# microsoft/timewarp

Measured on AMD Instinct MI355X. Metric: MH-accepted samples/sec (whole node), alanine-dipeptide kernel_transformer_nvp, higher is better.
Workload: dtype f16x3 (split-fp16 operands, 3 MFMAs per fp32 product, fp32 accumulate)

## Files before the change

### include/timewarp_hip.h

```cpp
#ifndef TIMEWARP_HIP_H
#define TIMEWARP_HIP_H

#include <stddef.h>
#include <stdint.h>

#ifdef __cplusplus
extern "C" {
#endif

#define TW_ABI_VERSION 8

typedef enum {
  TW_OK = 0,
  TW_ERR_INVALID = -1,
  TW_ERR_HIP = -2,
  TW_ERR_WORKSPACE = -3,
  TW_ERR_NO_DEVICE = -4
} tw_status;

typedef struct {
  int32_t variant;
  int32_t n_coupling;
  int32_t n_layers;
  int32_t d_model;
// ... 180 lines not shown
                           const tw_forcefield* ff, const tw_mh_options* opt, const tw_mh_draws* draws,
                           const int32_t* atom_types, const uint8_t* masked, int32_t n_atoms, const float* x_coords,
                           const float* x_velocs, float* cur_velocs, float* zy_coords, float* zy_velocs, float* u,
                           float* new_coords, float* new_velocs, float* out_stats, uint8_t* out_accepted, int32_t* result,
                           int64_t n_proposals, int64_t n_chains, void* workspace, int64_t workspace_bytes, void* stream);
int tw_mh_draw_chains(const tw_flow_desc* desc, const float* raw, const tw_mh_draws* draws, float* z_coords, float* z_velocs,
                      float* u, float* velocs, int64_t n_proposals, int64_t n_chains, int32_t n_atoms, void* stream);

int tw_chirality_changed(const float* coords, const int32_t* centres, const float* reference_signs,
                         int32_t n_centres, uint8_t* out_changed, int64_t n_rows, int32_t n_atoms,
                         void* stream);

int tw_profile_begin(void);
int tw_profile_end(double* total_ms, int64_t* launches);

int tw_probe_mfma_clock(int32_t workgroups, int32_t iters, int64_t* cycles, double* ms, void* stream);

const char* tw_last_netblock_kernel(void);

const char* tw_last_attention_kernel(void);

const char* tw_flow_selected_kernel(const tw_flow_desc* desc, int32_t n_atoms, int64_t n_rows, int32_t path);

int tw_flow_nonfinite(int32_t reset, int32_t* out_flag);

#define TW_DEBUG_EXP_NO_WEIGHT_DMA (1 << 0)
#define TW_DEBUG_EXP_NO_BARRIERS (1 << 1)
#define TW_DEBUG_DUMP_ATTENTION (1 << 2)
#define TW_DEBUG_COMPILED_CPP (1 << 3)
#define TW_DEBUG_SECTION_STAMPS (1 << 4)
#define TW_DEBUG_SEPARATE_COUPLING (1 << 5)
#define TW_DEBUG_EXP_DENSE_NO_SOFTMAX (1 << 6)
#define TW_DEBUG_EXP_DENSE_NO_QKV_LDS (1 << 7)
#define TW_DEBUG_KEEP_PADDING (1 << 10)
#define TW_DEBUG_EXP_DENSE_NO_ATTENTION (1 << 11)
#define TW_DEBUG_PER_SECTION (1 << 12)
#define TW_DEBUG_ENC_WITH_DUMPS (1 << 13)
#define TW_DEBUG_NEVER_WIDE (1 << 14)
#define TW_DEBUG_ALWAYS_WIDE (1 << 15)
#define TW_DEBUG_ALWAYS_NT4 (1 << 16)
#define TW_DEBUG_NEVER_NT4 (1 << 17)
#define TW_DEBUG_WIDE_FIVE_GROUP_WINDOWS (1 << 18)
#define TW_DEBUG_WIDE_XT_BYTE_STORES (1 << 19)
#define TW_DEBUG_NEVER_PAIRED (1 << 20)
#define TW_DEBUG_PER_OP_ROWWISE (1 << 21)
#define TW_DEBUG_ENERGY_MAIN_STREAM (1 << 22)
#define TW_DEBUG_ENERGY_SIDE_STREAM (1 << 23)
#define TW_DEBUG_PER_OP_UNFUSED (1 << 24)
#define TW_DEBUG_FOLD_GEMM_SEPARATE (1 << 25)
#define TW_DEBUG_FOLD_ONE_WG_PER_TILE (1 << 26)
#define TW_DEBUG_FOLD_LN_SEPARATE (1 << 27)
#define TW_DEBUG_IO_GEMM_PAIRS (1 << 28)
#define TW_DEBUG_TOKENS_NT3 (1 << 29)
#define TW_DEBUG_TOKENS_NT4 (1 << 30)
#define TW_DEBUG_SDPA_SCALAR (-0x7fffffff - 1)
int tw_debug_set_flags(int flags);

int tw_debug_netblock(const tw_flow_desc* desc, const float* raw, const float* packed,
                      int32_t coupling, int32_t net, const int32_t* atom_types,
                      const float* x_coords, const float* x_velocs, const uint8_t* masked,
                      int64_t n_cond, const float* z_other, int64_t n_rows, int32_t n_atoms,
                      int32_t path, float* dump, void* workspace, int64_t workspace_bytes,
                      void* stream);

#ifdef __cplusplus
}
// ... 3 lines not shown
```

### timewarp_amd/_lib.py

```python
from __future__ import annotations

import ctypes as C
import enum
import os
from typing import Optional

import torch

from . import build as _build

_LIB: Optional[C.CDLL] = None

TW_PATH_AUTO, TW_PATH_FUSED, TW_PATH_SIMPLE, TW_PATH_FUSED_H3, TW_PATH_FUSED_H1, TW_PATH_SIMPLE_H3 = 0, 1, 2, 3, 4, 5


class DebugFlag(enum.IntFlag):

    EXP_NO_WEIGHT_DMA = 1 << 0
    EXP_NO_BARRIERS = 1 << 1
    DUMP_ATTENTION = 1 << 2
    COMPILED_CPP = 1 << 3
    SECTION_STAMPS = 1 << 4
    SEPARATE_COUPLING = 1 << 5
    EXP_DENSE_NO_SOFTMAX = 1 << 6
    EXP_DENSE_NO_QKV_LDS = 1 << 7
    KEEP_PADDING = 1 << 10
    EXP_DENSE_NO_ATTENTION = 1 << 11
    PER_SECTION = 1 << 12
    ENC_WITH_DUMPS = 1 << 13
    NEVER_WIDE = 1 << 14
    ALWAYS_WIDE = 1 << 15
    ALWAYS_NT4 = 1 << 16
    NEVER_NT4 = 1 << 17
    WIDE_FIVE_GROUP_WINDOWS = 1 << 18
    WIDE_XT_BYTE_STORES = 1 << 19
    NEVER_PAIRED = 1 << 20
    PER_OP_ROWWISE = 1 << 21
    ENERGY_MAIN_STREAM = 1 << 22
    ENERGY_SIDE_STREAM = 1 << 23
    PER_OP_UNFUSED = 1 << 24
    FOLD_GEMM_SEPARATE = 1 << 25
    FOLD_ONE_WG_PER_TILE = 1 << 26
    FOLD_LN_SEPARATE = 1 << 27
    IO_GEMM_PAIRS = 1 << 28
    TOKENS_NT3 = 1 << 29
    TOKENS_NT4 = 1 << 30
    SDPA_SCALAR = 1 << 31


def debug_word(flags) -> int:
    word = int(flags) & 0xFFFFFFFF
    return word - (1 << 32) if word & (1 << 31) else word


class FlowDesc(C.Structure):

    _fields_ = [
        ("variant", C.c_int32),
        ("n_coupling", C.c_int32),
        ("n_layers", C.c_int32),
        ("d_model", C.c_int32),
        ("d_ff", C.c_int32),
        ("d_hidden", C.c_int32),
        ("d_emb", C.c_int32),
        ("n_heads", C.c_int32),
        ("d_rff", C.c_int32),
        ("n_elements", C.c_int32),
        ("pos_mod2", C.c_int32),
        ("displacement", C.c_int32),
        ("ignore_cond_velocity", C.c_int32),
        ("normalise", C.c_int32),
        ("ln_eps", C.c_float),
        ("cheb_order", C.c_int32),
        ("cheb_force_zero", C.c_int32),
        ("range_flag", C.c_void_p),
        ("max_radius", C.c_float),
        ("n_hidden", C.c_int32),
    ]


# ... 177 lines not shown
```

### timewarp_amd/csrc/tw_netblock_h3.hip

```cpp
#include <utility>
#include <vector>

#include "tw_common.h"

namespace tw {

typedef float f4 __attribute__((ext_vector_type(4)));
typedef _Float16 h8 __attribute__((ext_vector_type(8)));
typedef _Float16 h4 __attribute__((ext_vector_type(4)));
typedef unsigned u4 __attribute__((ext_vector_type(4)));
typedef unsigned u2 __attribute__((ext_vector_type(2)));

#define H3_NT 3
#define H3_FFN_SPLIT 4
#define H3_TOK (16 * H3_NT)
#define H3_XT 48
#define H3_XT_IMG 1536
#define H3_PAIR_BYTES 2048
#define H3_STAGE_PAIRS 4
#define H3_STAGE_TILE_BYTES 8192
#define H3_STAGE_BYTES 9216
#define H3_RING 5
#define H3_XT_BYTES (128 * H3_XT * 2)
#define H3_WAVE_LDS (2 * H3_XT_BYTES)
// ... 512 lines not shown
    *(h8*)(base + lane * 16) = hi;
    *(h8*)(base + 1024 + lane * 16) = lo;
  }
}

struct H3Params {
  const char* packed;
  int64_t net_stride_bytes;
  int64_t stages;
  int64_t side_in2b, side_layers, side_layer_size, side_out2b, side_scales;
  const float* emb;
  const int32_t* types;
  const float* xc;
  const float* xv;
  const float* z_other;
  const char* sfrag;
  int sfrag_shared;
  int64_t sf_variant_bytes;
  int windowed;
  const float* rff;
  int d_rff;
  int win[4];
  float* out[2];
  float* dump;
  int64_t n_rows, n_cond;
  int V, mpw, nblocks;
  int ng;
  int P;
  int H, n_layers, ff_chunks, hid_chunks, d_emb;
  float eps;
  int net_sel;
  int debug;
  const uint8_t* masked;
  PrevCoupling prev;
};
#define H3_OPS(...)                                                                                                    \
  : [cur] "+&s"(cur), [gn] "+&v"(gn) : [ring] "s"(ring), [wave] "s"(wave), [priv] "s"(priv_lds), __VA_ARGS__ :
#define H3_IN_WIDE [xt] "s"(xt_lds), [win] "s"(win)
#define H3_IN_MASK0 [m0l] "v"(m0l), [m0h] "v"(m0h)
#define H3_IN_MASK12 [m1l] "v"(m1l), [m1h] "v"(m1h), [m2l] "v"(m2l), [m2h] "v"(m2h)
#define H3_OPS_IO H3_OPS([chunks] "s"(chunks))
#define H3_IN_ATTN [heads] "s"(heads), [sf] "v"(sfp)
#define H3_OPS_ATTN H3_OPS(H3_IN_ATTN)
#define H3_OPS_ATTN_WIDE H3_OPS(H3_IN_ATTN, H3_IN_WIDE)
#define H3_OPS_ATTN_DENSE H3_OPS([sl] "s"(sl_lds), H3_IN_MASK0, H3_IN_MASK12)
#define H3_OPS_ENC_V                                                                                                   \
  H3_OPS([heads] "s"(heads), [chunks] "s"(chunks), [layers] "s"(layers), [sf] "v"(sfp), [sfstride] "s"(sfstride),      \
         [side] "v"(sidep), [sidestride] "s"(sidestride), [sl] "s"(sl_lds), [scales] "s"(scp), [eps] "s"(eps),        \
         [padm] "v"(padmask), [padt] "s"(pad_tiles), [dump] "v"(stamp_base), [stampen] "s"(stampen))
#define H3_IN_ENC_S_SF                                                                                                 \
  [heads] "s"(heads), [chunks] "s"(chunks), [layers] "s"(layers), [sf] "s"(sf_u), [sfstride] "s"(sfstride_lo),         \
      [sfstridehi] "s"(sfstride_hi)
#define H3_IN_ENC_S_SIDE                                                                                               \
  [side] "s"(side_u), [sidestride] "s"(sidestride32), [sl] "s"(sl_lds), [scales] "s"(scales_u), [eps] "s"(eps),        \
      [padm] "v"(padmask), [padt] "s"(pad_tiles), [dump] "s"(dump_u), [stampen] "s"(stampen)
#define H3_OPS_ENC_S H3_OPS(H3_IN_ENC_S_SF, H3_IN_ENC_S_SIDE)
#define H3_OPS_ENC_S_WIDE H3_OPS(H3_IN_ENC_S_SF, H3_IN_ENC_S_SIDE, H3_IN_WIDE)
#define H3_OPS_ENC_DENSE4 H3_OPS([chunks] "s"(chunks), [layers] "s"(layers), H3_IN_ENC_S_SIDE, H3_IN_MASK0)
#define H3_OPS_ENC_DENSE3 H3_OPS([chunks] "s"(chunks), [layers] "s"(layers), H3_IN_ENC_S_SIDE, H3_IN_MASK0, H3_IN_MASK12)
__device__ __forceinline__ void h3_load_sf4(const char* p, u4 (&r)[16]) {
  asm volatile(
      "global_load_dwordx4 %0, %16, off\n\t"
      "global_load_dwordx4 %1, %16, off offset:1024\n\t"
      "global_load_dwordx4 %2, %16, off offset:2048\n\t"
      "global_load_dwordx4 %3, %16, off offset:3072\n\t"
      "global_load_dwordx4 %4, %17, off\n\t"
// ... 31 lines not shown
  for (int jt = 0; jt < NT; ++jt) acc[jt] = mfma32(ah, b.l[jt], acc[jt]);
#pragma unroll
  for (int jt = 0; jt < NT; ++jt) acc[jt] = mfma32(al, b.h[jt], acc[jt]);
}

__device__ __forceinline__ void split_pair(float a, float b, unsigned& hi, unsigned& lo) {
  float ta, tb;
  asm("v_cvt_pk_f16_f32 %0, %4, %5\n\t"
      "v_fma_mix_f32 %2, %0, -1.0, %4 op_sel_hi:[1,0,0]\n\t"
      "v_fma_mix_f32 %3, %0, -1.0, %5 op_sel:[1,0,0] op_sel_hi:[1,0,0]\n\t"
      "v_cvt_pk_f16_f32 %1, %2, %3"
      : "=&v"(hi), "=&v"(lo), "=&v"(ta), "=&v"(tb)
      : "v"(a), "v"(b));
}

__device__ __forceinline__ void split8(const f4 a, const f4 b, h8& hi, h8& lo) {
  unsigned h0, h1, h2, h3, l0, l1, l2, l3;
  split_pair(a[0], a[1], h0, l0);
  split_pair(a[2], a[3], h1, l1);
  split_pair(b[0], b[1], h2, l2);
  split_pair(b[2], b[3], h3, l3);
  hi = __builtin_bit_cast(h8, (u4){h0, h1, h2, h3});
  lo = __builtin_bit_cast(h8, (u4){l0, l1, l2, l3});
}

__device__ __forceinline__ void split4(const f4 a, h4& hi, h4& lo) {
  unsigned h0, h1, l0, l1;
  split_pair(a[0], a[1], h0, l0);
  split_pair(a[2], a[3], h1, l1);
  hi = __builtin_bit_cast(h4, (u2){h0, h1});
  lo = __builtin_bit_cast(h4, (u2){l0, l1});
}

__device__ __forceinline__ void h3_swap16(float& a, float& b) {
  asm("s_nop 1\n\tv_permlane16_swap_b32 %0, %1" : "+v"(a), "+v"(b));
}
__device__ __forceinline__ void h3_swap32(float& a, float& b) {
  asm("s_nop 1\n\tv_permlane32_swap_b32 %0, %1" : "+v"(a), "+v"(b));
}
__device__ __forceinline__ float h3_quad_max(float v) {
  float a = v, b = v;
  h3_swap16(a, b);
  a = b = fmaxf(a, b);
  h3_swap32(a, b);
  return fmaxf(a, b);
}
__device__ __forceinline__ float h3_quad_sum(float v) {
  float a = v, b = v;
  h3_swap16(a, b);
  a = b = a + b;
  h3_swap32(a, b);
  return a + b;
}

__device__ __forceinline__ float h3_xor_sum(float v) { return h3_quad_sum(v); }

template <int NT, int KS>
__device__ __forceinline__ void to_bop(const f4 (&x)[2 * KS][NT], BOp<NT> (&b)[KS]) {
#pragma unroll
  for (int ks = 0; ks < KS; ++ks)
#pragma unroll
    for (int jt = 0; jt < NT; ++jt) split8(x[2 * ks][jt], x[2 * ks + 1][jt], b[ks].h[jt], b[ks].l[jt]);
}

__device__ __forceinline__ void h3_load_sf3(const char* p16, const char* p8, u4 (&a)[3], u4 (&b)[3], u2 (&c)[3], u2 (&d)[3]) {
  asm volatile(
// ... 283 lines not shown
      const char* src = (const char*)(side + p.side_layers) + lane * 16;
      char* dst = lds + SIDE_LDS_OFFSET;
#pragma unroll
      for (int i = 0; i < SIDE_CHUNKS; ++i)
        __builtin_amdgcn_global_load_lds((const __attribute__((address_space(1))) void*)(src + i * 1024),
                                         (__attribute__((address_space(3))) void*)(dst + i * 1024), 16, 0, 0);
    }
  }
  pipe.start_issue();

  const float sc_in2 = scales[1], sc_out2 = scales[2 + 3 * p.n_layers + 1];
  f4 bb_in2[8];
#pragma unroll
  for (int ot = 0; ot < 8; ++ot) bb_in2[ot] = *(const f4*)(side + p.side_in2b + 4 * g + 16 * ot);
  const f4 bb_out2 = *(const f4*)(side + p.side_out2b + 4 * g);

  int64_t tok_row[NT];
  int64_t tok_cond[NT];
  int tok_atom[NT];
  const unsigned inv_v = (65536u + (unsigned)p.P - 1u) / (unsigned)p.P;
  const bool cond_shared = p.n_cond == 1, cond_per_row = p.n_cond >= p.n_rows;
#pragma unroll
  for (int jt = 0; jt < NT; ++jt) {
    const int t = slot0 + 16 * jt + i16;
    const int q = (int)(((unsigned)t * inv_v) >> 16);
    const int64_t n = row0 + q;
    const int atom = t - q * p.P;
    const bool ok = active && q < p.mpw && n < p.n_rows && atom < p.V;
    tok_row[jt] = ok ? n : -1;
    tok_cond[jt] = !ok || cond_shared ? 0 : (cond_per_row ? n : n % p.n_cond);
    tok_atom[jt] = ok ? atom : 0;
  }
  float zo[NT][3];
  {
    float part[NT];
    bool bad = false;
#pragma unroll
    for (int jt = 0; jt < NT; ++jt) {
      const int64_t n = tok_row[jt];
      part[jt] = 0.f;
#pragma unroll
      for (int k = 0; k < 3; ++k) zo[jt][k] = 0.f;
      if (n < 0) continue;
      const int64_t idx = (n * p.V + tok_atom[jt]) * 3;
      if (p.prev.s_raw) {
        float ld = 0.f;
#pragma unroll
        for (int k = 0; k < 3; ++k) {
          const float sr = p.prev.s_raw[idx + k], shift = p.prev.t[idx + k];
          const float scale = expf(sr);
          bad |= !(isfinite(sr) && isfinite(shift));
          const float z = p.prev.z_in[idx + k];
          zo[jt][k] = p.prev.reverse ? (z - shift) / scale : z * scale + shift;
          ld += logf(scale);
        }
        part[jt] = p.masked[tok_cond[jt] * p.V + tok_atom[jt]] ? 0.f : ld;
        if (net == 0 && g == 0) {
#pragma unroll
          for (int k = 0; k < 3; ++k) p.prev.z_out[idx + k] = zo[jt][k];
        }
      } else {
#pragma unroll
        for (int k = 0; k < 3; ++k) zo[jt][k] = p.z_other[idx + k];
      }
    }
    if constexpr (WIDE) {
      if (p.prev.s_raw) {
// ... 9 lines not shown
        __builtin_amdgcn_s_barrier();
        if (net == 0 && wave == 0 && lane < p.mpw) {
          const int64_t n = row0 + lane;
          if (n < p.n_rows) {
            float acc = 0.f;
            for (int a = 0; a < p.V; ++a) acc += scr[lane * p.P + a];
            p.prev.delta_logp[n] -= p.prev.reverse ? -acc : acc;
          }
        }
        asm volatile("s_waitcnt lgkmcnt(0)" ::: "memory");
        __builtin_amdgcn_s_barrier();
      }
    } else
    if (p.prev.s_raw && net == 0) {
      if (bad) atomicOr(p.prev.nonfinite, 1);
      float* scr = (float*)xt_hi;
      if (g == 0) {
#pragma unroll
        for (int jt = 0; jt < NT; ++jt) scr[16 * jt + i16] = part[jt];
      }
      if (lane < p.mpw) {
        const int64_t n = (int64_t)blk * p.mpw + lane;
        if (active && n < p.n_rows) {
          float acc = 0.f;
          for (int a = 0; a < p.V; ++a) acc += scr[lane * p.V + a];
          p.prev.delta_logp[n] -= p.prev.reverse ? -acc : acc;
        }
      }
    }
  }
  const unsigned long long t_pro1 = (p.debug & TW_DEBUG_SECTION_STAMPS) ? __builtin_readcyclecounter() : 0ull;
  BOp<NT> u[KIN];
  const bool std_input = !RFF && p.d_emb == 32;
  if (std_input) {
#pragma unroll
    for (int jt = 0; jt < NT; ++jt) {
      const int64_t n = tok_row[jt];
      const int64_t ca = n < 0 ? 0 : tok_cond[jt] * p.V + tok_atom[jt];
      const int ty = n < 0 ? 0 : p.types[ca];
      const float* er = p.emb + ty * 32 + 4 * g;
      f4 e0, e1, m;
#pragma unroll
      for (int r = 0; r < 4; ++r) { e0[r] = er[r]; e1[r] = er[16 + r]; }
      const float c0 = p.xc[ca * 3], c1 = p.xc[ca * 3 + 1], c2 = p.xc[ca * 3 + 2];
      const float v0 = p.xv[ca * 3], v1 = p.xv[ca * 3 + 1], v2 = p.xv[ca * 3 + 2];
      m[0] = g == 0 ? c0 : g == 1 ? v1 : g == 2 ? zo[jt][2] : 0.f;
      m[1] = g == 0 ? c1 : g == 1 ? v2 : 0.f;
      m[2] = g == 0 ? c2 : g == 1 ? zo[jt][0] : 0.f;
      m[3] = g == 0 ? v0 : g == 1 ? zo[jt][1] : 0.f;
      if (n < 0) e0 = e1 = m = (f4){0.f, 0.f, 0.f, 0.f};
      split8(e0, e1, u[0].h[jt], u[0].l[jt]);
      split8(m, (f4){0.f, 0.f, 0.f, 0.f}, u[1].h[jt], u[1].l[jt]);
    }
  } else
#pragma unroll
  for (int jt = 0; jt < NT; ++jt) {
    const int64_t n = tok_row[jt];
    const int64_t c = tok_cond[jt];
    const int a = tok_atom[jt];
    const int ty = n < 0 ? 0 : p.types[c * p.V + a];
#pragma unroll
    for (int ks = 0; ks < KIN; ++ks)
#pragma unroll
      for (int e = 0; e < 8; ++e) {
        const int f = 32 * ks + 16 * (e / 4) + 4 * g + (e % 4);
        float val = 0.f;
        if (n >= 0) {
// ... 113 lines not shown
    }
  }
  unsigned padmask = 0;
#pragma unroll
  for (int jt = 0; jt < NT; ++jt) padmask |= (tok_row[jt] < 0 ? 1u : 0u) << jt;
  if (p.debug & TW_DEBUG_KEEP_PADDING) padmask = 0;
  unsigned pad_tiles = 0;
#pragma unroll
  for (int jt = 0; jt < NT; ++jt)
    if (__builtin_amdgcn_ballot_w64((padmask >> jt) & 1u) != 0ull) pad_tiles |= 1u << jt;
  pad_tiles = __builtin_amdgcn_readfirstlane(pad_tiles);
  auto zero_pad = [&]() {
#pragma unroll
    for (int jt = 0; jt < NT; ++jt) {
      if (!((pad_tiles >> jt) & 1u)) continue;
      const bool pad = (padmask >> jt) & 1u;
#pragma unroll
      for (int ft = 0; ft < 8; ++ft)
#pragma unroll
        for (int r = 0; r < 4; ++r) x[ft][jt][r] = pad ? 0.f : x[ft][jt][r];
    }
  };
  zero_pad();
  if (!(p.debug & TW_DEBUG_SECTION_STAMPS)) dump_x(x, 0);
  stamp(1);

  const char* sf_net = p.sfrag + (int64_t)(net * p.n_layers) * p.sf_variant_bytes +
                       (WIDE ? (int64_t)((p.sfrag_shared ? 0 : wg * 4) + wave) * p.H * ((int64_t)p.ng * NT * 2048)
                             : (p.sfrag_shared ? 0 : (int64_t)blk * p.H * NT * SF_BYTES));

  const float* sl = (const float*)(lds + SIDE_LDS_OFFSET);
  unsigned long long kvalid[NT];
  if constexpr (DENSE) {
#pragma unroll
    for (int jt = 0; jt < NT; ++jt) {
      unsigned long long m = 0ull;
      if (tok_row[jt] >= 0) {
        const int q = (16 * jt + i16) / p.V;
        const uint8_t* mk = p.masked + tok_cond[jt] * p.V;
        for (int a = 0; a < p.V; ++a) m |= mk[a] ? 0ull : (1ull << (q * p.V + a));
      }
      kvalid[jt] = m >> (4 * g);
    }
  }
  if constexpr (ENC) {
    static_assert(SIDE_CHUNKS == (DENSE ? 5 : 3), "gen_h3_enc_asm.py SIDE_CHUNKS");
    char* priv = (char*)xt_hi;
#pragma unroll
    for (int ft = 0; ft < 8; ++ft)
#pragma unroll
      for (int jt = 0; jt < NT; ++jt) *(f4*)(priv + (ft * NT + jt) * 1024 + lane * 16) = x[ft][jt];
    int cur = __builtin_amdgcn_readfirstlane(pipe.cur);
    const char* gn = pipe.gnext;
    const unsigned ring = (unsigned)(uintptr_t)(const __attribute__((address_space(3))) char*)lds;
    const unsigned priv_lds = (unsigned)(uintptr_t)(const __attribute__((address_space(3))) char*)priv;
    const unsigned sl_lds = (unsigned)(uintptr_t)(const __attribute__((address_space(3))) char*)(lds + SIDE_LDS_OFFSET);
    const int heads = __builtin_amdgcn_readfirstlane(p.H);
    const int chunks = __builtin_amdgcn_readfirstlane(p.ff_chunks);
    const int layers = __builtin_amdgcn_readfirstlane(p.n_layers);
    const char* sfp = sf_net;
    const int64_t sfstride = p.sf_variant_bytes;
    const char* sidep = (const char*)(side + p.side_layers) + lane * 16;
    const int64_t sidestride = (int64_t)p.side_layer_size * 4;
    const float* scp = scales + 2;
    const float eps = p.eps;
    const float* stamp_base = p.dump;
// ... 1036 lines not shown
    }
  }
  if constexpr (OUT) {
    const f4 bb = *(const f4*)(p.bias2 + 4 * g);
#pragma unroll
    for (int jt = 0; jt < NT; ++jt) {
      const f4 o = *(const f4*)(priv + jt * 1024 + lane * 16) * sc + bb;
      const int64_t t = t0 + 16 * jt + i16;
      if (g == 0 && t < p.n_tokens) {
        p.out[t * 3 + 0] = o[0];
        p.out[t * 3 + 1] = o[1];
        p.out[t * 3 + 2] = o[2];
      }
    }
  } else {
#pragma unroll
    for (int ot = 0; ot < 8; ++ot) {
      const f4 bb = *(const f4*)(p.bias2 + 4 * g + 16 * ot);
#pragma unroll
      for (int jt = 0; jt < NT; ++jt) {
        const int64_t t = t0 + 16 * jt + i16;
        if (t < p.n_tokens) *(f4*)(p.out + t * 128 + 16 * ot + 4 * g) = *(const f4*)(priv + (ot * NT + jt) * 1024 + lane * 16) * sc + bb;
      }
    }
  }
  asm volatile("s_waitcnt vmcnt(0)" ::: "memory");
}

struct H3Ws {
  float *s_out, *t_out;
  float *s_out2, *t_out2, *zc_alt, *zv_alt;
  char* sfrag;
  int64_t sf_variant_bytes;
  int64_t bytes;
};

static bool h3_layout(const tw_flow_desc& d, int V, int64_t n_rows, bool h1, FusedGeom* fg, H3Wide* wd, bool* wide) {
  *wide = h3_wide_choice(d, V, n_rows, h1);
  if (*wide) {
    h3_wide_geom(V, wd);
    fg->nt = wd->nt;
    fg->mpw = wd->mpwg;
    fg->tile_mask = 0;
    return true;
  }
  return fused_geom_nt(V, h3_nt4_choice(d, V, n_rows, h1) ? H3N4_NT : H3_NT, fg);
}

static H3Ws h3_ws(const tw_flow_desc& d, int64_t n_rows, int V, void* base, bool h1 = false, int force_layout = -1) {
  FusedGeom g;
  H3Wide wd;
  bool wide = false;
  h3_layout(d, V, n_rows, h1, &g, &wd, &wide);
  if (force_layout >= 0) {
    wide = force_layout == 1;
    if (wide) {
      if (!h3_wide_geom(V, &wd, false)) return H3Ws{};
      g.nt = H3_NT;
      g.mpw = wd.mpwg;
    } else if (!fused_geom_nt(V, force_layout == 2 ? H3N4_NT : H3_NT, &g)) {
      return H3Ws{};
    }
  }
  H3Ws w;
  char* p = (char*)base;
  auto take = [&](int64_t bytes) {
    char* r = p;
    p += (bytes + 255) / 256 * 256;
    return r;
  };
  const int64_t nblocks = (n_rows + g.mpw - 1) / g.mpw;
  w.s_out = (float*)take(n_rows * V * 3 * 4);
  w.t_out = (float*)take(n_rows * V * 3 * 4);
  w.s_out2 = (float*)take(n_rows * V * 3 * 4);
  w.t_out2 = (float*)take(n_rows * V * 3 * 4);
  w.zc_alt = (float*)take(n_rows * V * 3 * 4);
  w.zv_alt = (float*)take(n_rows * V * 3 * 4);
  const int64_t variants = d.cheb_order > 0 ? 2 * d.n_layers : 1;
  if (d.variant == 1) w.sf_variant_bytes = 0;
  else if (wide) w.sf_variant_bytes = nblocks * 4 * d.n_heads * h3w_frag_head(wd);
  else w.sf_variant_bytes = nblocks * d.n_heads * g.nt * (g.nt == 4 ? H3N4_SF_BYTES : H3_SF_BYTES);
  w.sfrag = take(wide ? (variants * nblocks * 4 * d.n_heads + 1) * (int64_t)H3W_FRAG_HEAD(H3W_NG6)
                      : variants * w.sf_variant_bytes + g.nt * (g.nt == 4 ? H3N4_SF_BYTES : H3_SF_BYTES));
  w.bytes = p - (char*)base;
  return w;
}

static bool h3_pair_enabled() {
  const int dbg = g_debug_flags;
  return !t_no_pair && !(dbg & (TW_DEBUG_COMPILED_CPP | TW_DEBUG_NEVER_PAIRED)) &&
         (!(dbg & (TW_DEBUG_DUMP_ATTENTION | TW_DEBUG_SECTION_STAMPS | TW_DEBUG_PER_SECTION)) || (dbg & TW_DEBUG_ENC_WITH_DUMPS));
}

static bool h3_windowed(const FusedGeom& fg, int V) {
  if (g_debug_flags & TW_DEBUG_COMPILED_CPP) return false;
  if (fg.mpw < 2) return false;
  const int end0 = (15 / V + 1) * V, start2 = (32 / V) * V;
  return end0 <= 32 && start2 >= 16;
}


int64_t h3_workspace_bytes(const tw_flow_desc& d, int64_t n_rows, int n_atoms) {
  int64_t b = 0;
  for (int layout = 0; layout < 3; ++layout)
    if (d.variant == 0 ? (layout == 0 ? h3_narrow_ok(d, n_atoms) : layout == 1 ? h3_wide_ok(n_atoms) : h3_nt4_ok(d, n_atoms, false))
                       : (layout == 0 ? !h3_nt4_ok(d, n_atoms, false) : layout == 2 && h3_nt4_ok(d, n_atoms, false))) {
      const int64_t x = h3_ws(d, n_rows, n_atoms, nullptr, false, layout).bytes;
      if (x > b) b = x;
    }
  return b;
}

static int h3_launch(const FlowArgs& a, const RawLayout& L, const FusedGeom& fg, int c, int net_sel, const float* z_other,
                     const char* sfrag, int64_t sf_variant_bytes, bool shared, float* s_out, float* t_out, float* dump,
                     const PrevCoupling& prev = PrevCoupling{}, bool dry = false) {
  const tw_flow_desc& d = *a.desc;
  const bool h1 = a.h1 != 0;
  const H3Geom g = h3_geom(d, h1);
  H3Params p;
  p.packed = (const char*)a.packed + (int64_t)(c * 2) * g.net_stride_bytes;
  p.net_stride_bytes = g.net_stride_bytes;
  p.stages = g.stages;
  p.side_in2b = g.side_in2b;
  p.side_layers = g.side_layers;
  p.side_layer_size = g.side_layer_size;
  p.side_out2b = g.side_out2b;
  p.side_scales = g.side_scales;
  p.emb = a.raw + L.emb;
  p.types = a.atom_types;
  p.xc = a.x_coords;
  p.xv = a.x_velocs;
  p.z_other = z_other;
  p.sfrag = sfrag;
  p.sfrag_shared = shared ? 1 : 0;
  p.sf_variant_bytes = sf_variant_bytes;
  H3Wide wd{};
  const bool wide = h3_wide_choice(d, a.n_atoms, a.n_rows, h1);
  if (wide) h3_wide_geom(a.n_atoms, &wd);
  p.d_rff = d.variant == 1 ? d.d_rff : 0;
  p.rff = p.d_rff > 0 ? a.raw + L.chain + (int64_t)c * L.coupling_size + L.rff : nullptr;
  p.windowed = (!wide && h3_windowed(fg, a.n_atoms)) ? 1 : 0;
  for (int i = 0; i < 4; ++i) p.win[i] = wide ? wd.win[i] : 0;
  p.out[0] = s_out;
  p.out[1] = t_out;
  p.dump = dump;
  p.n_rows = a.n_rows;
  p.n_cond = a.n_cond;
  p.V = a.n_atoms;
  p.P = wide ? wd.stride : a.n_atoms;
  p.ng = wide ? wd.ng : 0;
  p.mpw = fg.mpw;
  p.nblocks = (int)((a.n_rows + fg.mpw - 1) / fg.mpw);
  p.H = d.n_heads;
  p.n_layers = d.n_layers;
  p.ff_chunks = g.ff_chunks;
  p.hid_chunks = g.hid_chunks;
  p.d_emb = d.d_emb;
  p.eps = d.ln_eps;
  p.net_sel = net_sel;
  p.debug = g_debug_flags;
  p.masked = a.masked;
  p.prev = prev;
  const int wgs_per_net = wide ? p.nblocks : (p.nblocks + 3) / 4;
  unsigned grid = net_sel < 0 ? 8u * (unsigned)((wgs_per_net + 3) / 4) : (unsigned)wgs_per_net;
  int prc;
  if (!dry && (prc = profile_mark(a.stream, true))) return prc;
#define H3_STR2(...) #__VA_ARGS__
#define H3_STR(...) H3_STR2(__VA_ARGS__)
#define H3_LAUNCH(LDS, ...)                                                                                        \
  do {                                                                                                             \
    note_netblock_kernel("tw::netblock_h3_kernel<" H3_STR(__VA_ARGS__) ">");                                       \
    if (dry) return TW_OK;           \
    static LdsLimit lim;                                                                                           \
    if ((prc = lim.ensure((const void*)netblock_h3_kernel<__VA_ARGS__>, (int)(LDS)))) return prc;                  \
    hipLaunchKernelGGL((netblock_h3_kernel<__VA_ARGS__>), dim3(grid), dim3(256), (LDS), a.stream, p);              \
  } while (0)
  const bool per_section = ((dump != nullptr || (g_debug_flags & (TW_DEBUG_DUMP_ATTENTION | TW_DEBUG_SECTION_STAMPS | TW_DEBUG_PER_SECTION))) &&
                            !(g_debug_flags & TW_DEBUG_ENC_WITH_DUMPS)) ||
                           d.n_layers < 1;
  const bool cpp = (g_debug_flags & TW_DEBUG_COMPILED_CPP) != 0;
  if (wide && wd.nt == H3N4_NT) {
    TW_REQUIRE(d.variant == 0 && !per_section && !cpp, "paired 64-token layout: the encoder-stack statement only");
    if (h1) H3_LAUNCH(H3N4_LDS_BYTES, 4, true, false, true, false, true, true, false);
    else H3_LAUNCH(H3N4_LDS_BYTES, 4, true, false, true, false, true, false, false);
  } else if (!wide && fg.nt == H3N4_NT && d.variant == 1) {
    TW_REQUIRE(!h1 && d.d_rff == 0 && !cpp, "dense model on 64-token waves: the split-fp16 build without position features");
    if (per_section) H3_LAUNCH(H3D4_LDS_BYTES, 4, true, true, false, false, false, false, false);
    else H3_LAUNCH(H3D4_LDS_BYTES, 4, true, true, false, false, true, false, false);
  } else if (!wide && fg.nt == H3N4_NT) {
    TW_REQUIRE(d.variant == 0, "64-token waves: kernel attention");
    if (h1 && per_section) H3_LAUNCH(H3N4_LDS_BYTES, 4, true, false, false, false, false, true, false);
    else if (h1) H3_LAUNCH(H3N4_LDS_BYTES, 4, true, false, false, false, true, true, false);
    else if (cpp) H3_LAUNCH(H3N4_LDS_BYTES, 4, false, false, false, false, false, false, false);
    else if (per_section) H3_LAUNCH(H3N4_LDS_BYTES, 4, true, false, false, false, false, false, false);
// ... 59 lines not shown
    if (shmw > (size_t)64 * 1024) {
      static LdsLimit limw;
      int lrc;
      if ((lrc = limw.ensure((const void*)h3w_score_frag_kernel, (int)H3_SF_LDS_MAX))) return lrc;
    }
    H3WideWin win;
    for (int i = 0; i < 4; ++i) win.w[i] = wd.win[i];
    hipLaunchKernelGGL(h3w_score_frag_kernel, dim3((unsigned)nblocks, (unsigned)d.n_heads, (unsigned)basis.n_variants), dim3(512),
                       shmw, a.stream, a.x_coords, a.masked, lsw, d.n_heads, V, wd.stride, wd.ng, wd.mpwg, a.n_rows, a.n_cond, d.normalise, w.sfrag,
                       basis, vbw, V > 25 ? 1 : 0, win, wd.nt);
    TW_LAUNCH_CHECK();
    *variant_bytes = vbw;
    return TW_OK;
  }
  const int64_t vb = basis.n_variants > 1 ? nblocks * d.n_heads * fg.nt * (fg.nt == 4 ? H3N4_SF_BYTES : H3_SF_BYTES) : 0;
  const unsigned nv = (unsigned)basis.n_variants;
  const float* ls = a.raw + L.lengthscales + (a.reverse ? d.n_heads : 0);
  const int win = h3_windowed(fg, V) ? 1 : 0;
  const size_t shm = h3_sf_lds_bytes(d.n_heads, V, fg.mpw);
  TW_REQUIRE(shm <= H3_SF_LDS_MAX, "score fragments: %zu bytes of LDS for %d atoms x %d heads", shm, V, d.n_heads);
  if (shm > (size_t)64 * 1024) {
    static LdsLimit lim;
    int lrc;
    if ((lrc = lim.ensure((const void*)h3_score_frag_kernel, (int)H3_SF_LDS_MAX))) return lrc;
  }
  hipLaunchKernelGGL(h3_score_frag_kernel, dim3((unsigned)nblocks, 1, nv), dim3(shared ? 1024 : 512), shm, a.stream, a.x_coords,
                     a.masked, ls, d.n_heads, V, fg.mpw, a.n_rows, a.n_cond, d.normalise, w.sfrag, basis, vb, win, V > 25 ? 1 : 0,
                     fg.nt);
  TW_LAUNCH_CHECK();
  *variant_bytes = vb;
  return TW_OK;
}

int flow_pass_h3(const FlowArgs& a) {
  const tw_flow_desc& d = *a.desc;
  NoPairScope no_pair(d.n_layers < 1);
  FusedGeom fg;
  H3Wide wdg;
  bool wide_layout = false;
  TW_REQUIRE(h3_layout(d, a.n_atoms, a.n_rows, a.h1 != 0, &fg, &wdg, &wide_layout) && !(wide_layout && d.variant != 0),
             "split-fp16 path: unsupported atom count %d", a.n_atoms);
  const RawLayout L = raw_layout(d);
  const H3Ws w = h3_ws(d, a.n_rows, a.n_atoms, a.ws, a.h1 != 0);
  TW_REQUIRE_WORKSPACE(w.bytes, a.ws_bytes);
  const bool shared = a.n_cond == 1;
  int rc;
  int64_t vb = 0;
  const bool kernel_attention = d.variant == 0;
  if (kernel_attention && d.cheb_order == 0 && (rc = h3_score_frags(a, L, fg, w, shared, 0, &vb))) return rc;
  float* caller[2] = {a.z_coords, a.z_velocs};
  float* cur[2] = {a.z_coords, a.z_velocs};
  float* alt[2] = {w.zc_alt, w.zv_alt};
  float* sbuf[2] = {w.s_out, w.s_out2};
  float* tbuf[2] = {w.t_out, w.t_out2};
  int* flag = flow_range_flag(d);
  TW_REQUIRE(flag != nullptr, "hipGetSymbolAddress(g_nonfinite) failed");
  PrevCoupling prev{};
  int tv = 0;
  if (g_debug_flags & TW_DEBUG_SEPARATE_COUPLING) {
    for (int i = 0; i < d.n_coupling; ++i) {
      const int c = a.reverse ? d.n_coupling - 1 - i : i;
      const bool positions = (c % 2) == d.pos_mod2;
      if (kernel_attention && d.cheb_order > 0 && (rc = h3_score_frags(a, L, fg, w, shared, c, &vb))) return rc;
      if ((rc = h3_launch(a, L, fg, c, -1, positions ? a.z_velocs : a.z_coords, w.sfrag, vb, shared, w.s_out, w.t_out, nullptr)))
        return rc;
      if ((rc = launch_coupling(w.s_out, w.t_out, a.masked, a.n_cond, positions ? a.z_coords : a.z_velocs, a.delta_logp,
                                a.n_rows, a.n_atoms, a.reverse, a.stream, nullptr, flag)))
        return rc;
    }
    return TW_OK;
  }
  for (int i = 0; i < d.n_coupling; ++i) {
    const int c = a.reverse ? d.n_coupling - 1 - i : i;
    const bool positions = (c % 2) == d.pos_mod2;
    tv = positions ? 0 : 1;
    const int ov = 1 - tv;
    if (prev.s_raw) {
      prev.z_in = cur[ov];
      prev.z_out = alt[ov];
    }
    if (kernel_attention && d.cheb_order > 0 && (rc = h3_score_frags(a, L, fg, w, shared, c, &vb))) return rc;
    if ((rc = h3_launch(a, L, fg, c, -1, cur[ov], w.sfrag, vb, shared, sbuf[i & 1], tbuf[i & 1], nullptr, prev))) return rc;
    if (prev.s_raw) std::swap(cur[ov], alt[ov]);
    prev = PrevCoupling{sbuf[i & 1], tbuf[i & 1], nullptr, nullptr, a.delta_logp, flag, a.reverse};
  }
  if ((rc = launch_coupling(prev.s_raw, prev.t, a.masked, a.n_cond, caller[tv], a.delta_logp, a.n_rows, a.n_atoms, a.reverse,
                            a.stream, cur[tv], flag)))
    return rc;
  const int ov = 1 - tv;
  if (cur[ov] != caller[ov])
    TW_HIP_CHECK(hipMemcpyAsync(caller[ov], cur[ov], (size_t)a.n_rows * a.n_atoms * 3 * sizeof(float), hipMemcpyDeviceToDevice,
                                a.stream));
  return TW_OK;
}

bool h3_ffn_tokens_supported(const tw_flow_desc& d) { return h3_supported(d, 22); }

int h3_ffn_tokens(const tw_flow_desc& d, const void* packed, int coupling, int net, int layer, float* h, int64_t n_tokens,
                  hipStream_t stream, float* scratch, int64_t scratch_floats, const void* split_stages) {
  TW_REQUIRE(packed && h3_ffn_tokens_supported(d), "FFN on the split-fp16 stream: unsupported model or no stream");
  const H3Geom g = h3_geom(d);
  const int64_t att_stages = d.variant == 1 ? 4LL * g.H : 8LL * g.H;
  const int64_t first = (int64_t)(g.in_a_stages + 2) * g.hid_chunks + (int64_t)layer * (att_stages + 4LL * g.ff_chunks) + att_stages;
  const char* net_base = (const char*)packed + (int64_t)(coupling * 2 + net) * g.net_stride_bytes;
  H3FfnParams p;
  p.stages = net_base + first * H3_STAGE_BYTES;
  p.side = (const float*)(net_base + g.stages * H3_STAGE_BYTES) + g.side_layers + (int64_t)layer * g.side_layer_size;
  p.h = h;
  p.n_tokens = n_tokens;
  p.ff_chunks = g.ff_chunks;
  p.eps = d.ln_eps;
  p.split = 1;
  p.parts = scratch;
  const int64_t wg3 = (n_tokens + 191) / 192, wg4 = (n_tokens + 255) / 256;
  const int cus = H3_CUS;
// ... 95 lines not shown
  TW_REQUIRE(wgs < (int64_t)1 << 31, "in / out MLP: %lld workgroups", (long long)wgs);
  constexpr int lds3 = H3_RING * H3_STAGE_BYTES + 4 * H3_WAVE_LDS, lds4 = H3N4_RING * H3_STAGE_BYTES + 4 * H3N4_WAVE_LDS;
  static LdsLimit lim[4];
  const void* fn[4] = {(const void*)h3_io_tokens_kernel<false, 3>, (const void*)h3_io_tokens_kernel<false, 4>,
                       (const void*)h3_io_tokens_kernel<true, 3>, (const void*)h3_io_tokens_kernel<true, 4>};
  const int which = (out ? 2 : 0) + (four ? 1 : 0);
  const int lds = four ? lds4 : lds3;
  int rc;
  if ((rc = lim[which].ensure(fn[which], lds))) return rc;
  switch (which) {
    case 0: hipLaunchKernelGGL((h3_io_tokens_kernel<false, 3>), dim3((unsigned)wgs), dim3(256), lds, stream, p); break;
    case 1: hipLaunchKernelGGL((h3_io_tokens_kernel<false, 4>), dim3((unsigned)wgs), dim3(256), lds, stream, p); break;
    case 2: hipLaunchKernelGGL((h3_io_tokens_kernel<true, 3>), dim3((unsigned)wgs), dim3(256), lds, stream, p); break;
    default: hipLaunchKernelGGL((h3_io_tokens_kernel<true, 4>), dim3((unsigned)wgs), dim3(256), lds, stream, p); break;
  }
  TW_LAUNCH_CHECK();
  return TW_OK;
}

int h3_selected_kernel(const tw_flow_desc& d, int n_atoms, int64_t n_rows, bool h1) {
  NoPairScope no_pair(d.n_layers < 1);
  FlowArgs a{};
  a.desc = &d;
  a.n_rows = n_rows;
  a.n_cond = 1;
  a.n_atoms = n_atoms;
  a.h1 = h1 ? 1 : 0;
  FusedGeom fg;
  H3Wide wdg;
  bool wide_layout = false;
  TW_REQUIRE(h3_layout(d, n_atoms, n_rows, h1, &fg, &wdg, &wide_layout) && !(wide_layout && d.variant != 0),
             "split-fp16 path: unsupported atom count %d", n_atoms);
  const RawLayout L = raw_layout(d);
  return h3_launch(a, L, fg, 0, -1, nullptr, nullptr, 0, true, nullptr, nullptr, nullptr, PrevCoupling{}, true);
}

int debug_netblock_h3(const FlowArgs& a, int c, int net, const float* z_other, float* dump) {
  const tw_flow_desc& d = *a.desc;
  NoPairScope no_pair;
  FusedGeom fg;
  H3Wide wdg;
  bool wide_layout = false;
  TW_REQUIRE(h3_layout(d, a.n_atoms, a.n_rows, a.h1 != 0, &fg, &wdg, &wide_layout) && !(wide_layout && d.variant != 0),
             "split-fp16 path: unsupported atom count %d", a.n_atoms);
  const RawLayout L = raw_layout(d);
  const H3Ws w = h3_ws(d, a.n_rows, a.n_atoms, a.ws, a.h1 != 0);
  TW_REQUIRE_WORKSPACE(w.bytes, a.ws_bytes);
  const bool shared = a.n_cond == 1;
  int rc;
  int64_t vb = 0;
  if (d.variant == 0 && (rc = h3_score_frags(a, L, fg, w, shared, c, &vb))) return rc;
  return h3_launch(a, L, fg, c, net, z_other, w.sfrag, vb, shared, w.s_out, w.t_out, dump);
}

}

#undef H3_OPS
#undef H3_IN_WIDE
#undef H3_IN_MASK0
#undef H3_IN_MASK12
#undef H3_OPS_IO
#undef H3_IN_ATTN
#undef H3_OPS_ATTN
#undef H3_OPS_ATTN_WIDE
#undef H3_OPS_ATTN_DENSE
#undef H3_OPS_ENC_V
#undef H3_IN_ENC_S_SF
#undef H3_IN_ENC_S_SIDE
#undef H3_OPS_ENC_S
#undef H3_OPS_ENC_S_WIDE
#undef H3_OPS_ENC_DENSE4
#undef H3_OPS_ENC_DENSE3
```

Before: 158.5.

## Precompute split-fp16 conditioning image once per flow pass and reuse across couplings

Adds a small kernel that runs once per flow pass and builds a per-token image holding the split-fp16 atom embedding, the conditioning coordinates and velocities, and the mask bit. Each coupling's fused netblock prologue then loads this image with vector loads instead of gathering the embedding and conditioning inputs and splitting them every time. The dense attention key mask is also derived from the image's mask bit by a ballot. The cost is an extra launch, extra workspace, and a larger, more complex prologue with more register pressure.

New measurement: 159.1 (median of 6 runs). No clear change (+0.4%).

```diff
diff --git a/include/timewarp_hip.h b/include/timewarp_hip.h
--- a/include/timewarp_hip.h
+++ b/include/timewarp_hip.h
@@ -236,6 +236,7 @@
 #define TW_DEBUG_SEPARATE_COUPLING (1 << 5)
 #define TW_DEBUG_EXP_DENSE_NO_SOFTMAX (1 << 6)
 #define TW_DEBUG_EXP_DENSE_NO_QKV_LDS (1 << 7)
+enum { TW_DEBUG_NO_COND_IMAGE = 1 << 8 };
 #define TW_DEBUG_KEEP_PADDING (1 << 10)
 #define TW_DEBUG_EXP_DENSE_NO_ATTENTION (1 << 11)
 #define TW_DEBUG_PER_SECTION (1 << 12)
diff --git a/timewarp_amd/_lib.py b/timewarp_amd/_lib.py
--- a/timewarp_amd/_lib.py
+++ b/timewarp_amd/_lib.py
@@ -46,6 +46,9 @@
     TOKENS_NT3 = 1 << 29
     TOKENS_NT4 = 1 << 30
     SDPA_SCALAR = 1 << 31
+
+
+DEBUG_NO_COND_IMAGE = 1 << 8
 
 
 def debug_word(flags) -> int:
diff --git a/timewarp_amd/csrc/tw_netblock_h3.hip b/timewarp_amd/csrc/tw_netblock_h3.hip
--- a/timewarp_amd/csrc/tw_netblock_h3.hip
+++ b/timewarp_amd/csrc/tw_netblock_h3.hip
@@ -568,6 +568,7 @@
   int net_sel;
   int debug;
   const uint8_t* masked;
+  const char* cimg;
   PrevCoupling prev;
 };
 #define H3_OPS(...)                                                                                                    \
@@ -665,6 +666,37 @@
   lo = __builtin_bit_cast(h4, (u2){l0, l1});
 }
 
+constexpr int H3_CIMG_TOKEN_BYTES = 256;
+__global__ void __launch_bounds__(256) h3_cond_image_kernel(const float* __restrict__ emb, const int32_t* __restrict__ types,
+                                                            const float* __restrict__ xc, const float* __restrict__ xv,
+                                                            const uint8_t* __restrict__ masked, int64_t n_tokens,
+                                                            char* __restrict__ img) {
+  const int64_t i = (int64_t)blockIdx.x * 256 + threadIdx.x;
+  const int64_t ca = i >> 2;
+  const int g = (int)(i & 3);
+  if (ca >= n_tokens) return;
+  const float* er = emb + types[ca] * 32 + 4 * g;
+  f4 e0, e1, m;
+#pragma unroll
+  for (int r = 0; r < 4; ++r) { e0[r] = er[r]; e1[r] = er[16 + r]; }
+  const float c0 = xc[ca * 3], c1 = xc[ca * 3 + 1], c2 = xc[ca * 3 + 2];
+  const float v0 = xv[ca * 3], v1 = xv[ca * 3 + 1], v2 = xv[ca * 3 + 2];
+  m[0] = g == 0 ? c0 : g == 1 ? v1 : 0.f;
+  m[1] = g == 0 ? c1 : g == 1 ? v2 : 0.f;
+  m[2] = g == 0 ? c2 : 0.f;
+  m[3] = g == 0 ? v0 : 0.f;
+  h8 h0, l0, h1, l1;
+  split8(e0, e1, h0, l0);
+  split8(m, (f4){0.f, 0.f, 0.f, 0.f}, h1, l1);
+  u4 h1w = __builtin_bit_cast(u4, h1);
+  h1w[3] = (unsigned)masked[ca] << 16;
+  u4* dst = (u4*)(img + i * 64);
+  dst[0] = __builtin_bit_cast(u4, h0);
+  dst[1] = __builtin_bit_cast(u4, l0);
+  dst[2] = h1w;
+  dst[3] = __builtin_bit_cast(u4, l1);
+}
+
 __device__ __forceinline__ void h3_swap16(float& a, float& b) {
   asm("s_nop 1\n\tv_permlane16_swap_b32 %0, %1" : "+v"(a), "+v"(b));
 }
@@ -1014,7 +1046,139 @@
     tok_atom[jt] = ok ? atom : 0;
   }
   float zo[NT][3];
-  {
+  const bool use_img = !RFF && p.cimg != nullptr;
+  u4 ci[NT][4];
+  float za[NT], zb[NT];
+  unsigned long long wave_keys = 0ull;
+  if (use_img) {
+    const bool pend = p.prev.s_raw != nullptr;
+    float sr[NT][3], sh[NT][3], zi[NT][3];
+    const float* zsrc = pend ? p.prev.z_in : p.z_other;
+    int64_t zidx[NT];
+    const u4* ip[NT];
+#pragma unroll
+    for (int jt = 0; jt < NT; ++jt) {
+      const int64_t ca = tok_cond[jt] * p.V + tok_atom[jt];
+      ip[jt] = (const u4*)(p.cimg + (ca * 4 + g) * 64);
+      zidx[jt] = tok_row[jt] < 0 ? 0 : (tok_row[jt] * p.V + tok_atom[jt]) * 3;
+    }
+#pragma unroll
+    for (int jt = 0; jt < NT; ++jt) {
+#pragma unroll
+      for (int k = 0; k < 4; ++k) ci[jt][k] = ip[jt][k];
+#pragma unroll
+      for (int k = 0; k < 3; ++k) zi[jt][k] = zsrc[zidx[jt] + k];
+    }
+    const int64_t ld_row = WIDE ? row0 + lane : (int64_t)blk * p.mpw + lane;
+    const bool ld_lane = pend && net == 0 && lane < p.mpw && ld_row < p.n_rows && (WIDE ? wave == 0 : active);
+    float dl0 = 0.f;
+    if (pend) {
+#pragma unroll
+      for (int jt = 0; jt < NT; ++jt)
+#pragma unroll
+        for (int k = 0; k < 3; ++k) {
+          sr[jt][k] = p.prev.s_raw[zidx[jt] + k];
+          sh[jt][k] = p.prev.t[zidx[jt] + k];
+        }
+      dl0 = p.prev.delta_logp[ld_lane ? ld_row : 0];
+    } else {
+#pragma unroll
+      for (int jt = 0; jt < NT; ++jt)
+#pragma unroll
+        for (int k = 0; k < 3; ++k) sr[jt][k] = sh[jt][k] = 0.f;
+    }
+#pragma unroll
+    for (int jt = 0; jt < NT; ++jt) {
+      const bool pad = tok_row[jt] < 0;
+#pragma unroll
+      for (int k = 0; k < 4; ++k)
+#pragma unroll
+        for (int r = 0; r < 4; ++r) ci[jt][k][r] = pad ? 0u : ci[jt][k][r];
+#pragma unroll
+      for (int k = 0; k < 3; ++k) zi[jt][k] = pad ? 0.f : zi[jt][k];
+    }
+    if constexpr (DENSE) {
+#pragma unroll
+      for (int jt = 0; jt < NT; ++jt) {
+        const bool key = tok_row[jt] >= 0 && ((ci[jt][2][3] >> 16) & 0xffu) == 0u;
+        wave_keys |= (__builtin_amdgcn_ballot_w64(key) & 0xffffull) << (16 * jt);
+      }
+    }
+    float part[NT];
+    bool bad = false;
+#pragma unroll
+    for (int jt = 0; jt < NT; ++jt) {
+      part[jt] = 0.f;
+      float z0 = zi[jt][0], z1 = zi[jt][1], z2 = zi[jt][2];
+      if (pend && tok_row[jt] >= 0) {
+        float ld = 0.f;
+        auto update = [&](int k) {
+          const float s_raw = sr[jt][k], shift = sh[jt][k];
+          const float scale = expf(s_raw);
+          bad |= !(isfinite(s_raw) && isfinite(shift));
+          const float z = zi[jt][k];
+          ld += logf(scale);
+          return p.prev.reverse ? (z - shift) / scale : z * scale + shift;
+        };
+        z0 = update(0);
+        z1 = update(1);
+        z2 = update(2);
+        part[jt] = ((ci[jt][2][3] >> 16) & 0xffu) ? 0.f : ld;
+        if (net == 0 && g == 0) {
+          float* zp = p.prev.z_out + (tok_row[jt] * p.V + tok_atom[jt]) * 3;
+          zp[0] = z0;
+          zp[1] = z1;
+          zp[2] = z2;
+        }
+      }
+      za[jt] = g == 1 ? z0 : z2;
+      zb[jt] = g == 1 ? z1 : 0.f;
+    }
+    auto atom_order_sum = [&](const float* row) {
+      float acc = 0.f;
+      int a = 0;
+      for (; a + 4 <= p.V; a += 4) {
+        const float v0 = row[a], v1 = row[a + 1], v2 = row[a + 2], v3 = row[a + 3];
+        acc += v0;
+        acc += v1;
+        acc += v2;
+        acc += v3;
+      }
+      for (; a < p.V; ++a) acc += row[a];
+      return acc;
+    };
+    if constexpr (WIDE) {
+      if (pend) {
+        float* scr = (float*)(lds + RING * H3_STAGE_BYTES);
+        if (net == 0) {
+          if (bad) atomicOr(p.prev.nonfinite, 1);
+          if (g == 0) {
+#pragma unroll
+            for (int jt = 0; jt < NT; ++jt) scr[slot0 + 16 * jt + i16] = part[jt];
+          }
+        }
+        asm volatile("s_waitcnt lgkmcnt(0)" ::: "memory");
+        __builtin_amdgcn_s_barrier();
+        if (ld_lane) {
+          const float acc = atom_order_sum(scr + lane * p.P);
+          p.prev.delta_logp[ld_row] = dl0 - (p.prev.reverse ? -acc : acc);
+        }
+        asm volatile("s_waitcnt lgkmcnt(0)" ::: "memory");
+        __builtin_amdgcn_s_barrier();
+      }
+    } else if (pend && net == 0) {
+      if (bad) atomicOr(p.prev.nonfinite, 1);
+      float* scr = (float*)xt_hi;
+      if (g == 0) {
+#pragma unroll
+        for (int jt = 0; jt < NT; ++jt) scr[16 * jt + i16] = part[jt];
+      }
+      if (ld_lane) {
+        const float acc = atom_order_sum(scr + lane * p.V);
+        p.prev.delta_logp[ld_row] = dl0 - (p.prev.reverse ? -acc : acc);
+      }
+    }
+  } else {
     float part[NT];
     bool bad = false;
 #pragma unroll
@@ -1090,7 +1254,25 @@
   const unsigned long long t_pro1 = (p.debug & TW_DEBUG_SECTION_STAMPS) ? __builtin_readcyclecounter() : 0ull;
   BOp<NT> u[KIN];
   const bool std_input = !RFF && p.d_emb == 32;
-  if (std_input) {
+  if (use_img) {
+    if constexpr (!RFF) {
+#pragma unroll
+      for (int jt = 0; jt < NT; ++jt) {
+        unsigned zh, zl;
+        split_pair(za[jt], zb[jt], zh, zl);
+        u4 h = ci[jt][2], l = ci[jt][3];
+        h[0] = g == 2 ? zh : h[0];
+        l[0] = g == 2 ? zl : l[0];
+        h[1] = g == 1 ? zh : h[1];
+        l[1] = g == 1 ? zl : l[1];
+        h[3] &= 0x0000ffffu;
+        u[0].h[jt] = __builtin_bit_cast(h8, ci[jt][0]);
+        u[0].l[jt] = __builtin_bit_cast(h8, ci[jt][1]);
+        u[1].h[jt] = __builtin_bit_cast(h8, h);
+        u[1].l[jt] = __builtin_bit_cast(h8, l);
+      }
+    }
+  } else if (std_input) {
 #pragma unroll
     for (int jt = 0; jt < NT; ++jt) {
       const int64_t n = tok_row[jt];
@@ -1270,6 +1452,17 @@
   const float* sl = (const float*)(lds + SIDE_LDS_OFFSET);
   unsigned long long kvalid[NT];
   if constexpr (DENSE) {
+    if (use_img) {
+#pragma unroll
+      for (int jt = 0; jt < NT; ++jt) {
+        unsigned long long m = 0ull;
+        if (tok_row[jt] >= 0) {
+          const int q = (16 * jt + i16) / p.V;
+          m = wave_keys & (p.V >= 64 ? ~0ull : ((1ull << p.V) - 1ull) << (q * p.V));
+        }
+        kvalid[jt] = m >> (4 * g);
+      }
+    } else
 #pragma unroll
     for (int jt = 0; jt < NT; ++jt) {
       unsigned long long m = 0ull;
@@ -2372,8 +2565,11 @@
   float *s_out2, *t_out2, *zc_alt, *zv_alt;
   char* sfrag;
   int64_t sf_variant_bytes;
+  char* cimg;
   int64_t bytes;
 };
+
+static bool h3_cond_image_ok(const tw_flow_desc& d) { return d.d_emb == 32 && !(d.variant == 1 && d.d_rff > 0); }
 
 static bool h3_layout(const tw_flow_desc& d, int V, int64_t n_rows, bool h1, FusedGeom* fg, H3Wide* wd, bool* wide) {
   *wide = h3_wide_choice(d, V, n_rows, h1);
@@ -2422,6 +2618,7 @@
   else w.sf_variant_bytes = nblocks * d.n_heads * g.nt * (g.nt == 4 ? H3N4_SF_BYTES : H3_SF_BYTES);
   w.sfrag = take(wide ? (variants * nblocks * 4 * d.n_heads + 1) * (int64_t)H3W_FRAG_HEAD(H3W_NG6)
                       : variants * w.sf_variant_bytes + g.nt * (g.nt == 4 ? H3N4_SF_BYTES : H3_SF_BYTES));
+  w.cimg = h3_cond_image_ok(d) ? take(n_rows * V * H3_CIMG_TOKEN_BYTES) : nullptr;
   w.bytes = p - (char*)base;
   return w;
 }
@@ -2453,7 +2650,7 @@
 
 static int h3_launch(const FlowArgs& a, const RawLayout& L, const FusedGeom& fg, int c, int net_sel, const float* z_other,
                      const char* sfrag, int64_t sf_variant_bytes, bool shared, float* s_out, float* t_out, float* dump,
-                     const PrevCoupling& prev = PrevCoupling{}, bool dry = false) {
+                     const char* cimg, const PrevCoupling& prev = PrevCoupling{}, bool dry = false) {
   const tw_flow_desc& d = *a.desc;
   const bool h1 = a.h1 != 0;
   const H3Geom g = h3_geom(d, h1);
@@ -2500,6 +2697,7 @@
   p.net_sel = net_sel;
   p.debug = g_debug_flags;
   p.masked = a.masked;
+  p.cimg = cimg;
   p.prev = prev;
   const int wgs_per_net = wide ? p.nblocks : (p.nblocks + 3) / 4;
   unsigned grid = net_sel < 0 ? 8u * (unsigned)((wgs_per_net + 3) / 4) : (unsigned)wgs_per_net;
@@ -2625,6 +2823,20 @@
   return TW_OK;
 }
 
+static int h3_cond_image(const FlowArgs& a, const RawLayout& L, const H3Ws& w, const char** img) {
+  *img = nullptr;
+  if (!w.cimg || (g_debug_flags & TW_DEBUG_NO_COND_IMAGE)) return TW_OK;
+  const int64_t n_tokens = (a.n_cond < a.n_rows ? a.n_cond : a.n_rows) * a.n_atoms;
+  if (n_tokens <= 0) return TW_OK;
+  const int64_t blocks = (n_tokens * 4 + 255) / 256;
+  TW_REQUIRE(blocks < (int64_t)1 << 31, "conditioning image: %lld workgroups", (long long)blocks);
+  hipLaunchKernelGGL(h3_cond_image_kernel, dim3((unsigned)blocks), dim3(256), 0, a.stream, a.raw + L.emb, a.atom_types, a.x_coords,
+                     a.x_velocs, a.masked, n_tokens, w.cimg);
+  TW_LAUNCH_CHECK();
+  *img = w.cimg;
+  return TW_OK;
+}
+
 int flow_pass_h3(const FlowArgs& a) {
   const tw_flow_desc& d = *a.desc;
   NoPairScope no_pair(d.n_layers < 1);
@@ -2641,6 +2853,8 @@
   int64_t vb = 0;
   const bool kernel_attention = d.variant == 0;
   if (kernel_attention && d.cheb_order == 0 && (rc = h3_score_frags(a, L, fg, w, shared, 0, &vb))) return rc;
+  const char* cimg = nullptr;
+  if ((rc = h3_cond_image(a, L, w, &cimg))) return rc;
   float* caller[2] = {a.z_coords, a.z_velocs};
   float* cur[2] = {a.z_coords, a.z_velocs};
   float* alt[2] = {w.zc_alt, w.zv_alt};
@@ -2655,7 +2869,7 @@
       const int c = a.reverse ? d.n_coupling - 1 - i : i;
       const bool positions = (c % 2) == d.pos_mod2;
       if (kernel_attention && d.cheb_order > 0 && (rc = h3_score_frags(a, L, fg, w, shared, c, &vb))) return rc;
-      if ((rc = h3_launch(a, L, fg, c, -1, positions ? a.z_velocs : a.z_coords, w.sfrag, vb, shared, w.s_out, w.t_out, nullptr)))
+      if ((rc = h3_launch(a, L, fg, c, -1, positions ? a.z_velocs : a.z_coords, w.sfrag, vb, shared, w.s_out, w.t_out, nullptr, cimg)))
         return rc;
       if ((rc = launch_coupling(w.s_out, w.t_out, a.masked, a.n_cond, positions ? a.z_coords : a.z_velocs, a.delta_logp,
                                 a.n_rows, a.n_atoms, a.reverse, a.stream, nullptr, flag)))
@@ -2673,7 +2887,7 @@
       prev.z_out = alt[ov];
     }
     if (kernel_attention && d.cheb_order > 0 && (rc = h3_score_frags(a, L, fg, w, shared, c, &vb))) return rc;
-    if ((rc = h3_launch(a, L, fg, c, -1, cur[ov], w.sfrag, vb, shared, sbuf[i & 1], tbuf[i & 1], nullptr, prev))) return rc;
+    if ((rc = h3_launch(a, L, fg, c, -1, cur[ov], w.sfrag, vb, shared, sbuf[i & 1], tbuf[i & 1], nullptr, cimg, prev))) return rc;
     if (prev.s_raw) std::swap(cur[ov], alt[ov]);
     prev = PrevCoupling{sbuf[i & 1], tbuf[i & 1], nullptr, nullptr, a.delta_logp, flag, a.reverse};
   }
@@ -2835,7 +3049,7 @@
   TW_REQUIRE(h3_layout(d, n_atoms, n_rows, h1, &fg, &wdg, &wide_layout) && !(wide_layout && d.variant != 0),
              "split-fp16 path: unsupported atom count %d", n_atoms);
   const RawLayout L = raw_layout(d);
-  return h3_launch(a, L, fg, 0, -1, nullptr, nullptr, 0, true, nullptr, nullptr, nullptr, PrevCoupling{}, true);
+  return h3_launch(a, L, fg, 0, -1, nullptr, nullptr, 0, true, nullptr, nullptr, nullptr, nullptr, PrevCoupling{}, true);
 }
 
 int debug_netblock_h3(const FlowArgs& a, int c, int net, const float* z_other, float* dump) {
@@ -2853,7 +3067,9 @@
   int rc;
   int64_t vb = 0;
   if (d.variant == 0 && (rc = h3_score_frags(a, L, fg, w, shared, c, &vb))) return rc;
-  return h3_launch(a, L, fg, c, net, z_other, w.sfrag, vb, shared, w.s_out, w.t_out, dump);
+  const char* cimg = nullptr;
+  if ((rc = h3_cond_image(a, L, w, &cimg))) return rc;
+  return h3_launch(a, L, fg, c, net, z_other, w.sfrag, vb, shared, w.s_out, w.t_out, dump, cimg);
 }
 
 }
```
